# Sid-Rafilson-1617/poor-man-GPLVM

Measured on NVIDIA B200. Metric: EM time-bins x iters/s, higher is better.
Workload: dtype f32

## Files before the change

### poor_man_gplvm_b200/csrc/pmg_gemm_tc.cu

```cuda
#include "pmg_common.cuh"
#include "pmg_tc.cuh"
#include <cuda_bf16.h>

namespace pmg {

using namespace tc;

constexpr int TC_BM = 128;
constexpr int TC_BK = 64;
constexpr int TC_THREADS = 256;
constexpr int TC_A_BYTES = TC_BM * TC_BK * 2;

__global__ void counts_to_f16_kernel(int64_t T, int N, const float* __restrict__ y, int64_t ldy,
                                     __half* __restrict__ y16, int64_t ld16, int* __restrict__ inexact) {
  const int64_t total = T * ld16;
  int bad = 0;
  for (int64_t i = (int64_t)blockIdx.x * blockDim.x + threadIdx.x; i < total; i += (int64_t)gridDim.x * blockDim.x) {
    const int64_t t = i / ld16;
    const int n = (int)(i - t * ld16);
    float v = 0.f;
    if (n < N) v = y[(size_t)t * ldy + n];
    const __half h = __float2half_rn(v);
    if (__half2float(h) != v) ++bad;
    y16[i] = h;
// ... 687 lines not shown
        }
      }
    }
  } else if (warp == 1) {
    if (lane == 0) {
      int stage = 0; uint32_t phase = 0; int it = 0;
      for (int tile = blockIdx.x; tile < n_tiles; tile += gridDim.x, ++it) {
        const int buf = it & 1;
        const uint32_t acc_phase = (it >> 1) & 1;
        mbar_wait(&tempty[buf], acc_phase ^ 1);
        tc_fence_after();
        const uint32_t d_tmem = tmem_base + (uint32_t)(buf * BN);
        for (int kb = 0; kb < p.n_kblocks; ++kb) {
          mbar_wait(&full[stage], phase);
          tc_fence_after();
          const uint32_t sA = smem_u32(smem + (size_t)stage * stage_bytes);
#pragma unroll
          for (int pc = 0; pc < EM_PB; ++pc) {
            const uint32_t sB = sA + TC_A_BYTES + pc * b_bytes;
#pragma unroll
            for (int k = 0; k < TC_BK / 16; ++k) {
              const uint64_t ad = make_smem_desc(sA + k * 32, 16, 1024);
              const uint64_t bd = make_smem_desc(sB + k * 32, 16, 1024);
              mma_f16_ss(d_tmem, ad, bd, p.idesc, (kb | pc | k) != 0);
            }
          }
          mma_commit(&empty[stage]);
          if (++stage == p.stages) { stage = 0; phase ^= 1; }
        }
        mma_commit(&tfull[buf]);
      }
    }
  } else if (warp >= 4) {
    const int q = warp & 3;
    int it = 0;
    for (int tile = blockIdx.x; tile < n_tiles; tile += gridDim.x, ++it) {
      const int mt = tile / p.n_ntiles, nt = tile % p.n_ntiles;
      const int buf = it & 1;
      const uint32_t acc_phase = (it >> 1) & 1;
      mbar_wait(&tfull[buf], acc_phase);
      tc_fence_after();
      const int64_t t = (int64_t)mt * TC_BM + q * 32 + lane;
      const bool t_ok = t < p.T;
      const float lg = t_ok ? p.lgam[t] : 0.f;
      float* orow = p.ll + (size_t)(t_ok ? t : 0) * p.ldll;
      const uint32_t taddr = tmem_base + ((uint32_t)(q * 32) << 16) + (uint32_t)(buf * BN);
      const bool vec_ok = (p.ldll & 3) == 0;
      for (int c0 = 0; c0 < BN; c0 += 16) {
        uint32_t r[16];
        tmem_ld_x16(taddr + c0, r);
        tmem_ld_wait();
        const int k0 = nt * BN + c0;
        if (t_ok && k0 < p.K) {
          float v[16];
#pragma unroll
          for (int j = 0; j < 16; ++j) {
            const int k = k0 + j;
            float x = __uint_as_float(r[j]);
            if (k < p.K) {
              x = x - __ldg(p.lam_sum + k) - lg;
              if (p.ma_latent && __ldg(p.ma_latent + k) == 0.f) x = kVeryNegLL;
            }
            v[j] = x;
          }
          if (vec_ok && k0 + 16 <= p.K) {
#pragma unroll
            for (int j = 0; j < 16; j += 4)
              *reinterpret_cast<float4*>(orow + k0 + j) = make_float4(v[j], v[j + 1], v[j + 2], v[j + 3]);
          } else {
#pragma unroll
            for (int j = 0; j < 16; ++j)
              if (k0 + j < p.K) orow[k0 + j] = v[j];
          }
        }
      }
      tc_fence_before();
      mbar_arrive(&tempty[buf]);
    }
  }
  tc_fence_before();
  __syncthreads();
  if (warp == 2) { tc_fence_after(); tmem_dealloc(tmem_base, p.tmem_cols); }
}

static uint32_t pow2_cols(int c) {
  uint32_t v = 32;
  while ((int)v < c) v <<= 1;
  return v;
}

}

extern "C" int pmg_emission_tile_n(int K) {
  if (K <= 0) return 0;
  const int nt = (K + 255) / 256;
  int bn = (K + nt - 1) / nt;
  bn = (bn + 15) / 16 * 16;
  return bn;
}

extern "C" int pmg_counts_to_f16(int64_t T, int N, const float* y, int64_t ldy, void* y16, int64_t ld16,
                                 int* inexact_count, pmg_stream_t stream) {
  if (T <= 0 || N <= 0 || !y || !y16 || !inexact_count || ldy < N || ld16 < N || (ld16 & 7)) return PMG_ERR_BAD_ARG;
  cudaStream_t st = (cudaStream_t)stream;
  PMG_CUDA_CHECK(cudaMemsetAsync(inexact_count, 0, sizeof(int), st));
  pmg::counts_to_f16_kernel<<<148 * 8, 256, 0, st>>>(T, N, y, ldy, (__half*)y16, ld16, inexact_count);
  PMG_LAUNCH_CHECK();
  return PMG_OK;
}

extern "C" int pmg_counts_prepare(int64_t T, int N, const float* y, int64_t ldy, const float* ma_neuron, void* y16,
                                  int64_t ld16, int ones_col, int* inexact_count, float* lgam, float* ysum,
                                  pmg_stream_t stream) {
  if (T <= 0 || N <= 0 || !y || !y16 || !inexact_count || !lgam || ldy < N || (ld16 & 7)) return PMG_ERR_BAD_ARG;
  if (ld16 < N + (ones_col ? 1 : 0)) return PMG_ERR_BAD_ARG;
  cudaStream_t st = (cudaStream_t)stream;
  PMG_CUDA_CHECK(cudaMemsetAsync(inexact_count, 0, sizeof(int), st));
  const bool vec = (N & 3) == 0 && (ldy & 3) == 0 && ((uintptr_t)y & 15) == 0 && (!ma_neuron || ((uintptr_t)ma_neuron & 15) == 0);
  const unsigned grid = (unsigned)pmg::cdiv(T, 8);
  if (vec)
    pmg::counts_prepare_kernel<true><<<grid, 256, 0, st>>>(T, N, y, ldy, ma_neuron, (__half*)y16, ld16, ones_col,
                                                           inexact_count, lgam, ysum);
  else
    pmg::counts_prepare_kernel<false><<<grid, 256, 0, st>>>(T, N, y, ldy, ma_neuron, (__half*)y16, ld16, ones_col,
                                                            inexact_count, lgam, ysum);
  PMG_LAUNCH_CHECK();
  return PMG_OK;
}

extern "C" int pmg_counts_prepare_shifted(int64_t T, int N, int n_shift, const void* yT16, int64_t ld_src,
                                          const int* shifts, const float* ma_neuron, void* y16, int64_t ld16,
                                          float* lgam, pmg_stream_t stream) {
  if (T <= 0 || N <= 0 || n_shift <= 0 || !yT16 || !shifts || !y16 || !lgam) return PMG_ERR_BAD_ARG;
  if (ld_src < T || ld16 < N || (ld16 & 7)) return PMG_ERR_BAD_ARG;
  if ((uintptr_t)y16 & 15) return PMG_ERR_ALIGNMENT;
  const int64_t n_tiles = (T + pmg::SH_TT - 1) / pmg::SH_TT;
  if (n_tiles * n_shift > 0x7fffffffLL) return PMG_ERR_UNSUPPORTED_SHAPE;
  const bool vec = (N & 3) == 0 && (!ma_neuron || ((uintptr_t)ma_neuron & 15) == 0);
  const unsigned grid = (unsigned)(n_tiles * n_shift);
  cudaStream_t st = (cudaStream_t)stream;
  if (vec)
    pmg::counts_prepare_shifted_kernel<true><<<grid, pmg::SH_THREADS, 0, st>>>(
        T, N, n_tiles, (const __half*)yT16, ld_src, shifts, ma_neuron, (__half*)y16, ld16, lgam);
  else
    pmg::counts_prepare_shifted_kernel<false><<<grid, pmg::SH_THREADS, 0, st>>>(
        T, N, n_tiles, (const __half*)yT16, ld_src, shifts, ma_neuron, (__half*)y16, ld16, lgam);
  PMG_LAUNCH_CHECK();
  return PMG_OK;
}

extern "C" int pmg_emission_prepare_f16(int K, int N, const float* tuning, const float* ma_neuron, float dt,
                                        int Kpad, int64_t ld16, void* loglam16, float* lam_sum,
                                        pmg_stream_t stream) {
  if (K <= 0 || N <= 0 || !tuning || !loglam16 || !lam_sum || Kpad < K || ld16 < N || (ld16 & 7)) return PMG_ERR_BAD_ARG;
  pmg::emission_prepare_f16_kernel<<<Kpad, 128, 0, (cudaStream_t)stream>>>(K, N, tuning, ma_neuron, dt, Kpad, ld16,
                                                                          (__half*)loglam16, lam_sum);
  PMG_LAUNCH_CHECK();
  return PMG_OK;
}

extern "C" int pmg_emission_poisson_f16(int64_t T, int N, int K, const void* y16, int64_t ld16,
                                        const void* loglam16, int Kpad, const float* lam_sum, const float* lgam,
                                        const float* ma_latent, float* ll, int64_t ldll, pmg_stream_t stream) {
  using namespace pmg;
  if (T <= 0 || N <= 0 || K <= 0 || !y16 || !loglam16 || !lam_sum || !lgam || !ll) return PMG_ERR_BAD_ARG;
  if (ld16 < N || (ld16 & 7) || ldll < K) return PMG_ERR_BAD_ARG;
  if (((uintptr_t)y16 & 15) || ((uintptr_t)loglam16 & 15)) return PMG_ERR_ALIGNMENT;
  const int BN = pmg_emission_tile_n(K);
  const int n_ntiles = (K + BN - 1) / BN;
  if (Kpad != n_ntiles * BN) return PMG_ERR_BAD_ARG;
  if (T > ((int64_t)1 << 31) - 256) return PMG_ERR_UNSUPPORTED_SHAPE;

  CUtensorMap tmA, tmB;
  int rc = make_tmap_f16(&tmA, y16, (uint64_t)T, (uint64_t)ld16, (uint64_t)ld16, TC_BM);
  if (rc) return PMG_ERR_UNSUPPORTED_SHAPE;
  rc = make_tmap_f16(&tmB, loglam16, (uint64_t)EM_PB * Kpad, (uint64_t)ld16, (uint64_t)ld16, (uint32_t)BN);
  if (rc) return PMG_ERR_UNSUPPORTED_SHAPE;

  EmissionTcParams p;
  p.T = T; p.K = K; p.Kpad = Kpad; p.BN = BN;
  p.n_kblocks = (int)((ld16 + TC_BK - 1) / TC_BK);
  p.n_mtiles = (int)((T + TC_BM - 1) / TC_BM);
  p.n_ntiles = n_ntiles;
  p.stagger = 0;
  p.idesc = make_idesc_f16(TC_BM, BN, 0, 0, 0);
  p.tmem_cols = pow2_cols(2 * BN);
  p.lam_sum = lam_sum; p.lgam = lgam; p.ma_latent = ma_latent; p.ll = ll; p.ldll = ldll;
  p.ep_nbuf = 0;
  cudaStream_t st = (cudaStream_t)stream;
  int dev = 0, sms = 0;
  PMG_CUDA_CHECK(cudaGetDevice(&dev));
  PMG_CUDA_CHECK(cudaDeviceGetAttribute(&sms, cudaDevAttrMultiProcessorCount, dev));
  const size_t smem_max = 227 * 1024;

  bool paired = (ldll & 3) == 0 && ((uintptr_t)ll & 15) == 0;
  if (paired && (BN % 16) == 0 && T >= 4 * TC_BM) {
    const uint32_t stage_bytes = EM_MI * TC_A_BYTES + EM_PB * (BN / 2) * TC_BK * 2;
    const size_t fixed = 1024  + 256  + (size_t)((Kpad + 3) & ~3) * sizeof(float);
    int nbuf = 2, stages = 0;
    for (; nbuf >= 1; --nbuf) {
      const size_t stg_bytes = (size_t)8 * nbuf * EP_BUF_BYTES;
      stages = fixed + stg_bytes < smem_max ? (int)((smem_max - fixed - stg_bytes) / stage_bytes) : 0;
      if (stages >= 3) break;
    }
    if (nbuf < 1) { nbuf = 1; }
    if (stages >= 2) {
      if (stages > 6) stages = 6;
      EmissionTcParams p2 = p;
      p2.stages = stages;
      p2.ep_nbuf = nbuf;
      p2.idesc = make_idesc_f16(2 * TC_BM, BN, 0, 0, 0);
      CUtensorMap tmBh, tmC32, tmC16;
      rc = make_tmap_f16(&tmBh, loglam16, (uint64_t)EM_PB * Kpad, (uint64_t)ld16, (uint64_t)ld16, (uint32_t)(BN / 2));
      if (rc) return PMG_ERR_UNSUPPORTED_SHAPE;
      rc = make_tmap_f32(&tmC32, ll, (uint64_t)T, (uint64_t)K, (uint64_t)ldll, 32, 32);
      if (rc) return PMG_ERR_UNSUPPORTED_SHAPE;
      rc = make_tmap_f32(&tmC16, ll, (uint64_t)T, (uint64_t)K, (uint64_t)ldll, 32, 16);
      if (rc) return PMG_ERR_UNSUPPORTED_SHAPE;
      const size_t smem = (size_t)stages * stage_bytes + (size_t)8 * nbuf * EP_BUF_BYTES + fixed;
      PMG_CUDA_CHECK(cudaFuncSetAttribute(emission_tc2_kernel, cudaFuncAttributeMaxDynamicSharedMemorySize, (int)smem));
      PMG_CUDA_CHECK(cudaFuncSetAttribute(emission_tc2_kernel, cudaFuncAttributeNonPortableClusterSizeAllowed, 0));
      cudaLaunchConfig_t cfg = {};
      cudaLaunchAttribute attr[1];
      attr[0].id = cudaLaunchAttributeClusterDimension;
      attr[0].val.clusterDim.x = 2; attr[0].val.clusterDim.y = 1; attr[0].val.clusterDim.z = 1;
      cfg.blockDim = dim3(EM_THREADS); cfg.dynamicSmemBytes = smem; cfg.stream = st;
      cfg.attrs = attr; cfg.numAttrs = 1;
      cfg.gridDim = dim3((unsigned)(sms & ~1));
      static size_t occ_smem = 0;
      static int occ_clusters = 0, occ_dev = -1;
      static cudaError_t occ_err = cudaSuccess;
      if (occ_smem != smem || occ_dev != dev) {
        occ_dev = dev;
        occ_err = cudaOccupancyMaxActiveClusters(&occ_clusters, emission_tc2_kernel, &cfg);
        occ_smem = smem;
      }
      const int max_clusters = occ_clusters;
      const cudaError_t oe = occ_err;
      const int n_units2 = ((p.n_mtiles + 2 * EM_MI - 1) / (2 * EM_MI)) * p.n_ntiles;
      if (oe == cudaSuccess && max_clusters >= 1) {
        int n_cl = max_clusters < n_units2 ? max_clusters : n_units2;
        if (n_cl > sms / 2) n_cl = sms / 2;
        cfg.gridDim = dim3((unsigned)(2 * n_cl));
        PMG_CUDA_CHECK(cudaLaunchKernelEx(&cfg, emission_tc2_kernel, tmA, tmBh, tmC32, tmC16, p2));
        return PMG_OK;
      }
      (void)cudaGetLastError();
    }
  }
  if (paired) {
    const uint32_t stage_bytes = EM_MI * TC_A_BYTES + EM_PB * BN * TC_BK * 2;
    const size_t fixed = 1024  + 256  + (size_t)((Kpad + 3) & ~3) * sizeof(float);
    int nbuf = 2;
    int stages = 0;
    for (; nbuf >= 1; --nbuf) {
      const size_t stg_bytes = (size_t)8 * nbuf * EP_BUF_BYTES;
      stages = fixed + stg_bytes < smem_max ? (int)((smem_max - fixed - stg_bytes) / stage_bytes) : 0;
      if (stages >= 2) break;
    }
    if (stages < 2) {
      paired = false;
    } else {
      if (stages > 6) stages = 6;
      p.stages = stages;
      p.ep_nbuf = nbuf;
      CUtensorMap tmC32, tmC16;
      rc = make_tmap_f32(&tmC32, ll, (uint64_t)T, (uint64_t)K, (uint64_t)ldll, 32, 32);
      if (rc) return PMG_ERR_UNSUPPORTED_SHAPE;
      rc = make_tmap_f32(&tmC16, ll, (uint64_t)T, (uint64_t)K, (uint64_t)ldll, 32, 16);
      if (rc) return PMG_ERR_UNSUPPORTED_SHAPE;
      const size_t smem = (size_t)stages * stage_bytes + (size_t)8 * nbuf * EP_BUF_BYTES + fixed;
      PMG_CUDA_CHECK(cudaFuncSetAttribute(emission_tc_kernel, cudaFuncAttributeMaxDynamicSharedMemorySize, (int)smem));
      const int n_units = ((p.n_mtiles + EM_MI - 1) / EM_MI) * p.n_ntiles;
      emission_tc_kernel<<<n_units < sms ? n_units : sms, EM_THREADS, smem, st>>>(tmA, tmB, tmC32, tmC16, p);
      PMG_LAUNCH_CHECK();
      return PMG_OK;
    }
  }
  {
    const uint32_t stage_bytes = TC_A_BYTES + EM_PB * BN * TC_BK * 2;
    int stages = (int)((225 * 1024) / stage_bytes);
    if (stages > 2) stages = 2;
    if (stages < 2) return PMG_ERR_UNSUPPORTED_SHAPE;
    p.stages = stages;
    const size_t smem = (size_t)stages * stage_bytes + 1024  + 256 ;
    PMG_CUDA_CHECK(cudaFuncSetAttribute(emission_tc_kernel_v1, cudaFuncAttributeMaxDynamicSharedMemorySize, (int)smem));
    const int n_tiles = p.n_mtiles * p.n_ntiles;
    emission_tc_kernel_v1<<<n_tiles < sms ? n_tiles : sms, TC_THREADS, smem, st>>>(tmA, tmB, p);
    PMG_LAUNCH_CHECK();
  }
  return PMG_OK;
}

namespace pmg {

constexpr int AT_BKT = 32;
constexpr int AT_BOX_BYTES = AT_BKT * 128;
constexpr int AT_PG = 2;

struct AtbTcParams {
  int64_t T, t_per_split;
  int64_t g_lo_row;
  int K, N, BN, n_mtiles, n_ntiles, splits, stages;
  uint32_t tmem_cols;
  float* partial;
};

template <int PA, int FMT>
__global__ void __launch_bounds__(TC_THREADS, 1)
atb_tc_kernel(const __grid_constant__ CUtensorMap tmY, const __grid_constant__ CUtensorMap tmY1,
              const __grid_constant__ CUtensorMap tmG, const __grid_constant__ CUtensorMap tmG1,
              const AtbTcParams p) {
  extern __shared__ __align__(1024) uint8_t smem_raw[];
  uint8_t* smem = reinterpret_cast<uint8_t*>((reinterpret_cast<uintptr_t>(smem_raw) + 1023) & ~(uintptr_t)1023);
  const int mp = blockIdx.x, nt = blockIdx.y, sp = blockIdx.z;
  const int n_mi = (2 * mp + 1 < p.n_mtiles) ? 2 : 1;
  const int k_base = nt * p.BN;
  int bn = p.K - k_base;
  bn = (bn + 63) / 64 * 64;
  if (bn > p.BN) bn = p.BN;
  const int n_boxes_b = bn / 64;
  const uint32_t a_tile_bytes = 2 * AT_BOX_BYTES;
  const uint32_t a_bytes = 2 * PA * a_tile_bytes;
  const uint32_t b_piece_bytes = (uint32_t)(p.BN / 64) * AT_BOX_BYTES;
  const uint32_t stage_bytes = a_bytes + AT_PG * b_piece_bytes;
  uint64_t* full = reinterpret_cast<uint64_t*>(smem + (size_t)p.stages * stage_bytes);
  uint64_t* empty = full + p.stages;
  uint64_t* tfull = empty + p.stages;
  uint32_t* tmem_slot = reinterpret_cast<uint32_t*>(tfull + 1);

  const int warp = threadIdx.x >> 5, lane = threadIdx.x & 31;
  if (threadIdx.x == 0) {
    for (int s = 0; s < p.stages; ++s) { mbar_init(&full[s], 1); mbar_init(&empty[s], 1); }
    mbar_init(tfull, 1);
    fence_barrier_init();
  }
  if (warp == 0 && lane == 0) { tma_prefetch_desc(&tmY); tma_prefetch_desc(&tmG); tma_prefetch_desc(&tmG1); }
  if (warp == 2) { tmem_alloc(tmem_slot, p.tmem_cols); tmem_relinquish(); }
  tc_fence_before();
  __syncthreads();
  tc_fence_after();
  const uint32_t tmem_base = *tmem_slot;

  const int64_t t_begin = (int64_t)sp * p.t_per_split;
  int64_t t_end = t_begin + p.t_per_split;
  if (t_end > p.T) t_end = p.T;
  const int n_tb = t_end > t_begin ? (int)((t_end - t_begin + AT_BKT - 1) / AT_BKT) : 0;
  const uint32_t tx_bytes = (uint32_t)(n_mi * PA) * a_tile_bytes + AT_PG * (uint32_t)n_boxes_b * AT_BOX_BYTES;

  if (warp == 0) {
    if (lane == 0) {
      int stage = 0; uint32_t phase = 0;
      for (int tb = 0; tb < n_tb; ++tb) {
        mbar_wait(&empty[stage], phase ^ 1);
        uint8_t* sA = smem + (size_t)stage * stage_bytes;
        const int t0 = (int)(t_begin + (int64_t)tb * AT_BKT);
        mbar_arrive_expect_tx(&full[stage], tx_bytes);
        for (int mi = 0; mi < n_mi; ++mi) {
          const int m0 = (2 * mp + mi) * TC_BM;
#pragma unroll
          for (int pa = 0; pa < PA; ++pa) {
            const CUtensorMap* tm = pa == 0 ? &tmY : &tmY1;
            uint8_t* dst = sA + (mi * PA + pa) * a_tile_bytes;
            tma_load_2d(dst, tm, &full[stage], m0, t0);
            tma_load_2d(dst + AT_BOX_BYTES, tm, &full[stage], m0 + 64, t0);
          }
        }
        for (int pc = 0; pc < AT_PG; ++pc)
          for (int b = 0; b < n_boxes_b; ++b)
            tma_load_2d(sA + a_bytes + pc * b_piece_bytes + b * AT_BOX_BYTES, pc == 0 ? &tmG : &tmG1, &full[stage],
                        k_base + b * 64, (int)(pc * p.g_lo_row) + t0);
        if (++stage == p.stages) { stage = 0; phase ^= 1; }
      }
    }
  } else if (warp == 1) {
    if (lane == 0) {
      const uint32_t idesc = make_idesc_f16(TC_BM, bn, 1, 1, FMT);
      int stage = 0; uint32_t phase = 0;
      for (int tb = 0; tb < n_tb; ++tb) {
        mbar_wait(&full[stage], phase);
        tc_fence_after();
        const uint32_t sA = smem_u32(smem + (size_t)stage * stage_bytes);
        for (int mi = 0; mi < n_mi; ++mi) {
#pragma unroll
          for (int pa = 0; pa < PA; ++pa) {
#pragma unroll
            for (int pc = 0; pc < AT_PG; ++pc) {
              if (pa + pc > 1) continue;
              const uint32_t sB = sA + a_bytes + pc * b_piece_bytes;
#pragma unroll
              for (int k = 0; k < AT_BKT / 16; ++k) {
                const uint64_t ad = make_smem_desc(sA + (mi * PA + pa) * a_tile_bytes + k * 2048, AT_BOX_BYTES, 1024);
                const uint64_t bd = make_smem_desc(sB + k * 2048, AT_BOX_BYTES, 1024);
                mma_f16_ss(tmem_base + (uint32_t)(mi * p.BN), ad, bd, idesc, (tb | pa | pc | k) != 0);
              }
            }
          }
        }
        mma_commit(&empty[stage]);
        if (++stage == p.stages) { stage = 0; phase ^= 1; }
      }
      mma_commit(tfull);
    }
  } else if (warp >= 4) {
    const int q = warp & 3;
    float* out = p.partial + (size_t)sp * p.K * p.N;
    if (n_tb > 0) {
      mbar_wait(tfull, 0);
      tc_fence_after();
    }
    for (int mi = 0; mi < n_mi; ++mi) {
      const int n = (2 * mp + mi) * TC_BM + q * 32 + lane;
      const uint32_t taddr = tmem_base + ((uint32_t)(q * 32) << 16) + (uint32_t)(mi * p.BN);
      for (int c0 = 0; c0 < bn; c0 += 16) {
        uint32_t r[16];
        if (n_tb > 0) {
          tmem_ld_x16(taddr + c0, r);
          tmem_ld_wait();
        } else {
#pragma unroll
          for (int j = 0; j < 16; ++j) r[j] = 0u;
        }
        if (n < p.N) {
#pragma unroll
          for (int j = 0; j < 16; ++j) {
            const int k = k_base + c0 + j;
            if (k < p.K) out[(size_t)k * p.N + n] = __uint_as_float(r[j]);
          }
        }
      }
    }
  }
  tc_fence_before();
  __syncthreads();
  if (warp == 2) { tc_fence_after(); tmem_dealloc(tmem_base, p.tmem_cols); }
}

__global__ void split_bf16_kernel(int64_t T, int K, const float* __restrict__ src, int64_t lds,
                                  __nv_bfloat16* __restrict__ dst, int64_t ld16) {
  const int64_t total = T * ld16;
  for (int64_t i = (int64_t)blockIdx.x * blockDim.x + threadIdx.x; i < total; i += (int64_t)gridDim.x * blockDim.x) {
    const int64_t t = i / ld16;
    const int k = (int)(i - t * ld16);
    const float v = k < K ? src[(size_t)t * lds + k] : 0.f;
    const __nv_bfloat16 h = __float2bfloat16_rn(v);
    dst[i] = h;
    dst[total + i] = __float2bfloat16_rn(v - __bfloat162float(h));
  }
}

template <int HALF>
__global__ void __launch_bounds__(256) split_pieces_vec_kernel(int64_t T, int K8, const float* __restrict__ src,
                                                               int64_t lds, uint16_t* __restrict__ dst, int64_t ld16) {
  const int64_t total = T * (int64_t)K8;
  const size_t piece = (size_t)T * ld16;
  for (int64_t g = (int64_t)blockIdx.x * blockDim.x + threadIdx.x; g < total; g += (int64_t)gridDim.x * blockDim.x) {
    const int64_t t = g / K8;
    const int k = (int)(g - t * K8) * 8;
    const float4* sp = reinterpret_cast<const float4*>(src + (size_t)t * lds + k);
    const float4 a = __ldcs(sp), b = __ldcs(sp + 1);
    const float v[8] = {a.x, a.y, a.z, a.w, b.x, b.y, b.z, b.w};
    uint16_t hi[8], lo[8];
#pragma unroll
    for (int e = 0; e < 8; ++e) {
      if (HALF) {
        const __half h = __float2half_rn(v[e]);
        hi[e] = __half_as_ushort(h);
        lo[e] = __half_as_ushort(__float2half_rn(v[e] - __half2float(h)));
      } else {
        const __nv_bfloat16 h = __float2bfloat16_rn(v[e]);
        hi[e] = __bfloat16_as_ushort(h);
        lo[e] = __bfloat16_as_ushort(__float2bfloat16_rn(v[e] - __bfloat162float(h)));
      }
    }
    uint4 H, L;
    H.x = hi[0] | ((uint32_t)hi[1] << 16); H.y = hi[2] | ((uint32_t)hi[3] << 16);
    H.z = hi[4] | ((uint32_t)hi[5] << 16); H.w = hi[6] | ((uint32_t)hi[7] << 16);
    L.x = lo[0] | ((uint32_t)lo[1] << 16); L.y = lo[2] | ((uint32_t)lo[3] << 16);
    L.z = lo[4] | ((uint32_t)lo[5] << 16); L.w = lo[6] | ((uint32_t)lo[7] << 16);
    uint16_t* o = dst + (size_t)t * ld16 + k;
    *reinterpret_cast<uint4*>(o) = H;
    *reinterpret_cast<uint4*>(o + piece) = L;
  }
}

static bool split_vec_ok(int K, const void* src, int64_t lds, const void* dst, int64_t ld16) {
  return (K % 8) == 0 && K == ld16 && (lds % 4) == 0 && (((uintptr_t)src | (uintptr_t)dst) & 15) == 0;
}

__global__ void split_f16_kernel(int64_t T, int K, const float* __restrict__ src, int64_t lds,
                                 __half* __restrict__ dst, int64_t ld16) {
  const int64_t total = T * ld16;
  for (int64_t i = (int64_t)blockIdx.x * blockDim.x + threadIdx.x; i < total; i += (int64_t)gridDim.x * blockDim.x) {
    const int64_t t = i / ld16;
    const int k = (int)(i - t * ld16);
    const float v = k < K ? src[(size_t)t * lds + k] : 0.f;
    const __half h = __float2half_rn(v);
    dst[i] = h;
    dst[total + i] = __float2half_rn(v - __half2float(h));
  }
}

__global__ void split_reduce_kernel_tc(int splits, int64_t MN, const float* __restrict__ partial,
                                       float* __restrict__ C) {
  const int64_t i = (int64_t)blockIdx.x * blockDim.x + threadIdx.x;
  if (i >= MN) return;
  double s = 0.0;
  for (int z = 0; z < splits; ++z) s += (double)partial[(size_t)z * MN + i];
  C[i] = (float)s;
}

static void atb_tc_plan(int64_t T, int K, int N, int& BN, int& n_mtiles, int& n_ntiles, int& splits,
                        int64_t& t_per_split) {
  BN = K >= 256 ? 256 : (K + 63) / 64 * 64;
  n_ntiles = (K + BN - 1) / BN;
  n_mtiles = (N + TC_BM - 1) / TC_BM;
  const int tiles = ((n_mtiles + 1) / 2) * n_ntiles;
  splits = 148 / tiles;
  if (splits < 1) splits = 1;
  const int64_t max_splits = (T + 4 * AT_BKT - 1) / (4 * AT_BKT);
  if (splits > max_splits) splits = (int)max_splits;
  if (splits < 1) splits = 1;
  t_per_split = ((T + splits - 1) / splits + AT_BKT - 1) / AT_BKT * AT_BKT;
  splits = (int)((T + t_per_split - 1) / t_per_split);
}

}

extern "C" int pmg_split_f16(int64_t T, int K, const float* src, int64_t lds, void* dst16, int64_t ld16,
                             pmg_stream_t stream) {
  if (T <= 0 || K <= 0 || !src || !dst16 || lds < K || ld16 < K || (ld16 & 7)) return PMG_ERR_BAD_ARG;
  if (pmg::split_vec_ok(K, src, lds, dst16, ld16))
    pmg::split_pieces_vec_kernel<1><<<148 * 16, 256, 0, (cudaStream_t)stream>>>(T, K / 8, src, lds, (uint16_t*)dst16, ld16);
  else
    pmg::split_f16_kernel<<<148 * 8, 256, 0, (cudaStream_t)stream>>>(T, K, src, lds, (__half*)dst16, ld16);
  PMG_LAUNCH_CHECK();
  return PMG_OK;
}

extern "C" int64_t pmg_atb_f16_workspace_bytes(int64_t T, int K, int N) {
  if (T <= 0 || K <= 0 || N <= 0) return 0;
  int BN, nm, nn, splits; int64_t tps;
  pmg::atb_tc_plan(T, K, N, BN, nm, nn, splits, tps);
  return (int64_t)splits * K * N * (int64_t)sizeof(float);
}

extern "C" int pmg_split_bf16(int64_t T, int K, const float* src, int64_t lds, void* dst16, int64_t ld16,
                              pmg_stream_t stream) {
  if (T <= 0 || K <= 0 || !src || !dst16 || lds < K || ld16 < K || (ld16 & 7)) return PMG_ERR_BAD_ARG;
  if (pmg::split_vec_ok(K, src, lds, dst16, ld16))
    pmg::split_pieces_vec_kernel<0><<<148 * 16, 256, 0, (cudaStream_t)stream>>>(T, K / 8, src, lds, (uint16_t*)dst16, ld16);
  else
    pmg::split_bf16_kernel<<<148 * 8, 256, 0, (cudaStream_t)stream>>>(T, K, src, lds, (__nv_bfloat16*)dst16, ld16);
  PMG_LAUNCH_CHECK();
  return PMG_OK;
}

static int atb_pieces_launch(int64_t T, int K, int N, const void* g16, const void* g16_lo, int64_t ldg,
                             const void* y16, const void* y16_lo, int64_t ldy16, int fmt, float* yw, void* workspace,
                             int64_t workspace_bytes, pmg_stream_t stream);

extern "C" int pmg_atb_f16(int64_t T, int K, int N, const void* g16, int64_t ldg, const void* y16, int64_t ldy16,
                           float* yw, void* workspace, int64_t workspace_bytes, pmg_stream_t stream) {
  return atb_pieces_launch(T, K, N, g16, nullptr, ldg, y16, nullptr, ldy16, 0, yw, workspace, workspace_bytes, stream);
}

extern "C" int pmg_atb_bf16x2(int64_t T, int K, int N, const void* g16, int64_t ldg, const void* y16, int64_t ldy16,
                              float* out, void* workspace, int64_t workspace_bytes, pmg_stream_t stream) {
  if (!y16 || T <= 0) return PMG_ERR_BAD_ARG;
  const char* lo = (const char*)y16 + (size_t)T * (size_t)ldy16 * 2;
  return atb_pieces_launch(T, K, N, g16, nullptr, ldg, y16, lo, ldy16, 1, out, workspace, workspace_bytes, stream);
}

extern "C" int pmg_atb_bf16x2_pieces(int64_t T, int K, int N, const void* g_hi, const void* g_lo, int64_t ldg,
                                     const void* y_hi, const void* y_lo, int64_t ldy16, float* out, void* workspace,
                                     int64_t workspace_bytes, pmg_stream_t stream) {
  if (!g_hi || !g_lo || !y_hi || !y_lo || T <= 0) return PMG_ERR_BAD_ARG;
  return atb_pieces_launch(T, K, N, g_hi, g_lo, ldg, y_hi, y_lo, ldy16, 1, out, workspace, workspace_bytes, stream);
}

static int atb_pieces_launch(int64_t T, int K, int N, const void* g16, const void* g16_lo, int64_t ldg,
                             const void* y16, const void* y16_lo, int64_t ldy16, int fmt, float* yw, void* workspace,
                             int64_t workspace_bytes, pmg_stream_t stream) {
  using namespace pmg;
  if (T <= 0 || K <= 0 || N <= 0 || !g16 || !y16 || !yw) return PMG_ERR_BAD_ARG;
  if (ldg < K || (ldg & 7) || ldy16 < N || (ldy16 & 7)) return PMG_ERR_BAD_ARG;
  if (((uintptr_t)g16 & 15) || ((uintptr_t)y16 & 15) || ((uintptr_t)g16_lo & 15)) return PMG_ERR_ALIGNMENT;
  if ((int64_t)AT_PG * T > ((int64_t)1 << 31) - 256) return PMG_ERR_UNSUPPORTED_SHAPE;
  AtbTcParams p;
  atb_tc_plan(T, K, N, p.BN, p.n_mtiles, p.n_ntiles, p.splits, p.t_per_split);
  if (!workspace || workspace_bytes < (int64_t)p.splits * K * N * (int64_t)sizeof(float)) return PMG_ERR_WORKSPACE;
  p.T = T; p.K = K; p.N = N; p.partial = (float*)workspace;
  const int PA = y16_lo ? 2 : 1;
  if (y16_lo && ((uintptr_t)y16_lo & 15)) return PMG_ERR_ALIGNMENT;
  const uint32_t stage_bytes = 4 * PA * AT_BOX_BYTES + AT_PG * (p.BN / 64) * AT_BOX_BYTES;
  int stages = (int)((200 * 1024) / stage_bytes);
  if (stages > 8) stages = 8;
  if (stages < 2) return PMG_ERR_UNSUPPORTED_SHAPE;
  p.stages = stages;
  p.tmem_cols = pow2_cols(2 * p.BN);

  CUtensorMap tmY, tmY1, tmG, tmG1;
  int rc = make_tmap_f16(&tmY, y16, (uint64_t)T, (uint64_t)ldy16, (uint64_t)ldy16, AT_BKT);
  if (rc) return PMG_ERR_UNSUPPORTED_SHAPE;
  rc = make_tmap_f16(&tmY1, y16_lo ? y16_lo : y16, (uint64_t)T, (uint64_t)ldy16, (uint64_t)ldy16, AT_BKT);
  if (rc) return PMG_ERR_UNSUPPORTED_SHAPE;
  rc = make_tmap_f16(&tmG, g16, (uint64_t)(g16_lo ? 1 : AT_PG) * T, (uint64_t)ldg, (uint64_t)ldg, AT_BKT);
  if (rc) return PMG_ERR_UNSUPPORTED_SHAPE;
  tmG1 = tmG;
  p.g_lo_row = T;
  if (g16_lo) {
    rc = make_tmap_f16(&tmG1, g16_lo, (uint64_t)T, (uint64_t)ldg, (uint64_t)ldg, AT_BKT);
    if (rc) return PMG_ERR_UNSUPPORTED_SHAPE;
    p.g_lo_row = 0;
  }
  const size_t smem = (size_t)stages * stage_bytes + 1024 + 256;
  cudaStream_t st = (cudaStream_t)stream;
  dim3 grid((p.n_mtiles + 1) / 2, p.n_ntiles, p.splits);
  if (PA == 1 && fmt == 0) {
    PMG_CUDA_CHECK(cudaFuncSetAttribute(atb_tc_kernel<1, 0>, cudaFuncAttributeMaxDynamicSharedMemorySize, (int)smem));
    atb_tc_kernel<1, 0><<<grid, TC_THREADS, smem, st>>>(tmY, tmY1, tmG, tmG1, p);
  } else if (PA == 2 && fmt == 1) {
    PMG_CUDA_CHECK(cudaFuncSetAttribute(atb_tc_kernel<2, 1>, cudaFuncAttributeMaxDynamicSharedMemorySize, (int)smem));
    atb_tc_kernel<2, 1><<<grid, TC_THREADS, smem, st>>>(tmY, tmY1, tmG, tmG1, p);
  } else {
    return PMG_ERR_BAD_ARG;
  }
  PMG_LAUNCH_CHECK();
  const int64_t MN = (int64_t)K * N;
  split_reduce_kernel_tc<<<cdiv(MN, 256), 256, 0, st>>>(p.splits, MN, p.partial, yw);
  PMG_LAUNCH_CHECK();
  return PMG_OK;
}

int64_t pmg_atb_tc_workspace_bytes(int64_t, int, int) { return 0; }
int pmg_atb_tc_launch(int64_t, int, int, const float*, int64_t, const float*, int64_t, float*, int64_t, void*,
                      int64_t, cudaStream_t) {
  return PMG_ERR_UNSUPPORTED_SHAPE;
}
```

### poor_man_gplvm_b200/csrc/pmg_tc.cuh

```cuda
#pragma once
#include <cuda.h>
#include <cuda_fp16.h>
#include <cuda_runtime.h>
#include <stdint.h>

namespace pmg {
namespace tc {

__device__ __forceinline__ uint32_t smem_u32(const void* p) {
  return static_cast<uint32_t>(__cvta_generic_to_shared(p));
}

__device__ __forceinline__ void mbar_init(uint64_t* bar, uint32_t count) {
  asm volatile("mbarrier.init.shared::cta.b64 [%0], %1;" ::"r"(smem_u32(bar)), "r"(count) : "memory");
}
__device__ __forceinline__ void fence_barrier_init() {
  asm volatile("fence.mbarrier_init.release.cluster;" ::: "memory");
}
__device__ __forceinline__ void mbar_arrive_expect_tx(uint64_t* bar, uint32_t bytes) {
  asm volatile("mbarrier.arrive.expect_tx.shared::cta.b64 _, [%0], %1;" ::"r"(smem_u32(bar)), "r"(bytes)
               : "memory");
}
__device__ __forceinline__ void mbar_arrive(uint64_t* bar) {
  asm volatile("mbarrier.arrive.shared::cta.b64 _, [%0];" ::"r"(smem_u32(bar)) : "memory");
}
__device__ __forceinline__ bool mbar_try_wait(uint64_t* bar, uint32_t parity) {
  uint32_t ok;
  asm volatile(
      "{\n\t.reg .pred p;\n\t"
      "mbarrier.try_wait.parity.shared::cta.b64 p, [%1], %2;\n\t"
      "selp.u32 %0, 1, 0, p;\n\t}"
      : "=r"(ok)
      : "r"(smem_u32(bar)), "r"(parity)
      : "memory");
  return ok != 0;
}
__device__ __forceinline__ void mbar_wait(uint64_t* bar, uint32_t parity) {
  while (!mbar_try_wait(bar, parity)) { }
}

__device__ __forceinline__ void tma_prefetch_desc(const CUtensorMap* m) {
  asm volatile("prefetch.tensormap [%0];" ::"l"(reinterpret_cast<uint64_t>(m)) : "memory");
}
__device__ __forceinline__ void tma_load_2d(void* smem_dst, const CUtensorMap* m, uint64_t* bar, int c_inner,
                                            int c_outer) {
  asm volatile(
      "cp.async.bulk.tensor.2d.shared::cluster.global.mbarrier::complete_tx::bytes [%0], [%1, {%3, %4}], [%2];"
      ::"r"(smem_u32(smem_dst)), "l"(reinterpret_cast<uint64_t>(m)), "r"(smem_u32(bar)), "r"(c_inner), "r"(c_outer)
      : "memory");
}

__device__ __forceinline__ void tma_store_2d(const CUtensorMap* m, const void* smem_src, int c_inner, int c_outer) {
  asm volatile("cp.async.bulk.tensor.2d.global.shared::cta.bulk_group [%0, {%2, %3}], [%1];"
               ::"l"(reinterpret_cast<uint64_t>(m)), "r"(smem_u32(smem_src)), "r"(c_inner), "r"(c_outer)
               : "memory");
}
__device__ __forceinline__ void bulk_commit() { asm volatile("cp.async.bulk.commit_group;" ::: "memory"); }
template <int N>
__device__ __forceinline__ void bulk_wait_read() {
  asm volatile("cp.async.bulk.wait_group.read %0;" ::"n"(N) : "memory");
}
__device__ __forceinline__ void fence_proxy_async_smem() { asm volatile("fence.proxy.async.shared::cta;" ::: "memory"); }

__device__ __forceinline__ void tmem_alloc(uint32_t* smem_dst, uint32_t ncols) {
  asm volatile("tcgen05.alloc.cta_group::1.sync.aligned.shared::cta.b32 [%0], %1;" ::"r"(smem_u32(smem_dst)),
               "r"(ncols)
               : "memory");
}
__device__ __forceinline__ void tmem_relinquish() {
  asm volatile("tcgen05.relinquish_alloc_permit.cta_group::1.sync.aligned;" ::: "memory");
}
__device__ __forceinline__ void tmem_dealloc(uint32_t taddr, uint32_t ncols) {
  asm volatile("tcgen05.dealloc.cta_group::1.sync.aligned.b32 %0, %1;" ::"r"(taddr), "r"(ncols) : "memory");
}
__device__ __forceinline__ void tc_fence_before() { asm volatile("tcgen05.fence::before_thread_sync;" ::: "memory"); }
__device__ __forceinline__ void tc_fence_after() { asm volatile("tcgen05.fence::after_thread_sync;" ::: "memory"); }

__device__ __forceinline__ void mma_f16_ss(uint32_t d_tmem, uint64_t adesc, uint64_t bdesc, uint32_t idesc,
                                           uint32_t accumulate) {
  asm volatile(
      "{\n\t.reg .pred p;\n\t"
      "setp.ne.b32 p, %4, 0;\n\t"
      "tcgen05.mma.cta_group::1.kind::f16 [%0], %1, %2, %3, p;\n\t}"
      ::"r"(d_tmem), "l"(adesc), "l"(bdesc), "r"(idesc), "r"(accumulate)
      : "memory");
}
__device__ __forceinline__ void mma_commit(uint64_t* bar) {
  asm volatile("tcgen05.commit.cta_group::1.mbarrier::arrive::one.shared::cluster.b64 [%0];" ::"r"(smem_u32(bar))
               : "memory");
}
__device__ __forceinline__ void tmem_ld_x16(uint32_t taddr, uint32_t (&r)[16]) {
  asm volatile(
      "tcgen05.ld.sync.aligned.32x32b.x16.b32 {%0, %1, %2, %3, %4, %5, %6, %7, %8, %9, %10, %11, %12, %13, %14, %15}, "
      "[%16];"
      : "=r"(r[0]), "=r"(r[1]), "=r"(r[2]), "=r"(r[3]), "=r"(r[4]), "=r"(r[5]), "=r"(r[6]), "=r"(r[7]), "=r"(r[8]),
        "=r"(r[9]), "=r"(r[10]), "=r"(r[11]), "=r"(r[12]), "=r"(r[13]), "=r"(r[14]), "=r"(r[15])
      : "r"(taddr)
      : "memory");
}
__device__ __forceinline__ void tmem_ld_x16_of32(uint32_t taddr, uint32_t (&r)[32]) {
  asm volatile(
      "tcgen05.ld.sync.aligned.32x32b.x16.b32 {%0, %1, %2, %3, %4, %5, %6, %7, %8, %9, %10, %11, %12, %13, %14, %15}, "
      "[%16];"
      : "=r"(r[0]), "=r"(r[1]), "=r"(r[2]), "=r"(r[3]), "=r"(r[4]), "=r"(r[5]), "=r"(r[6]), "=r"(r[7]), "=r"(r[8]),
        "=r"(r[9]), "=r"(r[10]), "=r"(r[11]), "=r"(r[12]), "=r"(r[13]), "=r"(r[14]), "=r"(r[15])
      : "r"(taddr)
      : "memory");
}
__device__ __forceinline__ void tmem_ld_x32(uint32_t taddr, uint32_t (&r)[32]) {
  asm volatile(
      "tcgen05.ld.sync.aligned.32x32b.x32.b32 {%0, %1, %2, %3, %4, %5, %6, %7, %8, %9, %10, %11, %12, %13, %14, %15, "
      "%16, %17, %18, %19, %20, %21, %22, %23, %24, %25, %26, %27, %28, %29, %30, %31}, [%32];"
      : "=r"(r[0]), "=r"(r[1]), "=r"(r[2]), "=r"(r[3]), "=r"(r[4]), "=r"(r[5]), "=r"(r[6]), "=r"(r[7]), "=r"(r[8]),
        "=r"(r[9]), "=r"(r[10]), "=r"(r[11]), "=r"(r[12]), "=r"(r[13]), "=r"(r[14]), "=r"(r[15]), "=r"(r[16]),
        "=r"(r[17]), "=r"(r[18]), "=r"(r[19]), "=r"(r[20]), "=r"(r[21]), "=r"(r[22]), "=r"(r[23]), "=r"(r[24]),
        "=r"(r[25]), "=r"(r[26]), "=r"(r[27]), "=r"(r[28]), "=r"(r[29]), "=r"(r[30]), "=r"(r[31])
      : "r"(taddr)
      : "memory");
}
__device__ __forceinline__ void tmem_ld_wait() { asm volatile("tcgen05.wait::ld.sync.aligned;" ::: "memory"); }

__device__ __forceinline__ uint32_t cluster_ctarank() {
  uint32_t r;
  asm volatile("mov.u32 %0, %%cluster_ctarank;" : "=r"(r));
  return r;
}
__device__ __forceinline__ void cluster_sync_all() {
  asm volatile("barrier.cluster.arrive.release.aligned;\n\tbarrier.cluster.wait.acquire.aligned;" ::: "memory");
}
__device__ __forceinline__ void tmem_alloc2(uint32_t* smem_dst, uint32_t ncols) {
  asm volatile("tcgen05.alloc.cta_group::2.sync.aligned.shared::cta.b32 [%0], %1;" ::"r"(smem_u32(smem_dst)),
               "r"(ncols)
               : "memory");
}
__device__ __forceinline__ void tmem_relinquish2() {
  asm volatile("tcgen05.relinquish_alloc_permit.cta_group::2.sync.aligned;" ::: "memory");
}
__device__ __forceinline__ void tmem_dealloc2(uint32_t taddr, uint32_t ncols) {
  asm volatile("tcgen05.dealloc.cta_group::2.sync.aligned.b32 %0, %1;" ::"r"(taddr), "r"(ncols) : "memory");
}
__device__ __forceinline__ void mma_f16_ss2(uint32_t d_tmem, uint64_t adesc, uint64_t bdesc, uint32_t idesc,
                                            uint32_t accumulate) {
  const uint32_t z = 0;
  asm volatile(
      "{\n\t.reg .pred p;\n\t"
      "setp.ne.b32 p, %4, 0;\n\t"
      "tcgen05.mma.cta_group::2.kind::f16 [%0], %1, %2, %3, {%5, %5, %5, %5, %5, %5, %5, %5}, p;\n\t}"
      ::"r"(d_tmem), "l"(adesc), "l"(bdesc), "r"(idesc), "r"(accumulate), "r"(z)
      : "memory");
}
__device__ __forceinline__ void mma_commit2(uint64_t* bar, uint16_t cta_mask) {
  asm volatile("tcgen05.commit.cta_group::2.mbarrier::arrive::one.shared::cluster.multicast::cluster.b64 [%0], %1;"
               ::"r"(smem_u32(bar)), "h"(cta_mask)
               : "memory");
}
__device__ __forceinline__ void tma_load_2d_pair(void* smem_dst, const CUtensorMap* m, uint64_t* bar, int c_inner,
                                                 int c_outer) {
  asm volatile(
      "cp.async.bulk.tensor.2d.cta_group::2.shared::cluster.global.mbarrier::complete_tx::bytes [%0], [%1, {%3, %4}], [%2];"
      ::"r"(smem_u32(smem_dst)), "l"(reinterpret_cast<uint64_t>(m)), "r"(smem_u32(bar) & 0xFEFFFFFFu), "r"(c_inner),
        "r"(c_outer)
      : "memory");
}
__device__ __forceinline__ void mbar_arrive_cluster(uint64_t* bar, uint32_t cta) {
  asm volatile(
      "{\n\t.reg .b32 ra;\n\t"
      "mapa.shared::cluster.u32 ra, %0, %1;\n\t"
      "mbarrier.arrive.release.cluster.shared::cluster.b64 _, [ra];\n\t}"
      ::"r"(smem_u32(bar)), "r"(cta)
      : "memory");
}

__device__ __forceinline__ uint64_t make_smem_desc(uint32_t saddr, uint32_t lbo_bytes, uint32_t sbo_bytes) {
  uint64_t d = 0;
  d |= (uint64_t)((saddr >> 4) & 0x3FFF);
  d |= (uint64_t)((lbo_bytes >> 4) & 0x3FFF) << 16;
  d |= (uint64_t)((sbo_bytes >> 4) & 0x3FFF) << 32;
  d |= (uint64_t)1 << 46;
  d |= (uint64_t)2 << 61;
  return d;
}
__host__ __device__ constexpr uint32_t make_idesc_f16(int M, int N, int a_mn_major, int b_mn_major, int fmt) {
  return (1u << 4) | ((uint32_t)fmt << 7) | ((uint32_t)fmt << 10) | ((uint32_t)a_mn_major << 15) |
         ((uint32_t)b_mn_major << 16) | ((uint32_t)(N >> 3) << 17) | ((uint32_t)(M >> 4) << 24);
}

}

typedef CUresult (*PFN_encodeTiled)(CUtensorMap*, CUtensorMapDataType, cuuint32_t, void*, const cuuint64_t*,
                                    const cuuint64_t*, const cuuint32_t*, const cuuint32_t*, CUtensorMapInterleave,
                                    CUtensorMapSwizzle, CUtensorMapL2promotion, CUtensorMapFloatOOBfill);

inline PFN_encodeTiled get_encode_tiled() {
  static PFN_encodeTiled fn = nullptr;
  if (!fn) {
    void* p = nullptr;
    cudaDriverEntryPointQueryResult q;
    if (cudaGetDriverEntryPoint("cuTensorMapEncodeTiled", &p, cudaEnableDefault, &q) == cudaSuccess &&
        q == cudaDriverEntryPointSuccess)
      fn = reinterpret_cast<PFN_encodeTiled>(p);
  }
  return fn;
}

inline int make_tmap_f16(CUtensorMap* map, const void* base, uint64_t rows, uint64_t cols, uint64_t ld,
                         uint32_t box_rows) {
  PFN_encodeTiled enc = get_encode_tiled();
  if (!enc) return -100;
  cuuint64_t gdim[2] = {cols, rows};
  cuuint64_t gstr[1] = {ld * 2};
  cuuint32_t box[2] = {64, box_rows};
  cuuint32_t estr[2] = {1, 1};
  CUresult r = enc(map, CU_TENSOR_MAP_DATA_TYPE_FLOAT16, 2, const_cast<void*>(base), gdim, gstr, box, estr,
                   CU_TENSOR_MAP_INTERLEAVE_NONE, CU_TENSOR_MAP_SWIZZLE_128B, CU_TENSOR_MAP_L2_PROMOTION_L2_256B,
                   CU_TENSOR_MAP_FLOAT_OOB_FILL_NONE);
  return r == CUDA_SUCCESS ? 0 : -101;
}

inline int make_tmap_f32(CUtensorMap* map, const void* base, uint64_t rows, uint64_t cols, uint64_t ld,
                         uint32_t box_rows, uint32_t box_cols) {
  PFN_encodeTiled enc = get_encode_tiled();
  if (!enc) return -100;
  cuuint64_t gdim[2] = {cols, rows};
  cuuint64_t gstr[1] = {ld * 4};
  cuuint32_t box[2] = {box_cols, box_rows};
  cuuint32_t estr[2] = {1, 1};
  const CUtensorMapSwizzle sw = box_cols * 4 == 128 ? CU_TENSOR_MAP_SWIZZLE_128B
                              : box_cols * 4 == 64 ? CU_TENSOR_MAP_SWIZZLE_64B : CU_TENSOR_MAP_SWIZZLE_NONE;
  CUresult r = enc(map, CU_TENSOR_MAP_DATA_TYPE_FLOAT32, 2, const_cast<void*>(base), gdim, gstr, box, estr,
                   CU_TENSOR_MAP_INTERLEAVE_NONE, sw, CU_TENSOR_MAP_L2_PROMOTION_NONE,
                   CU_TENSOR_MAP_FLOAT_OOB_FILL_NONE);
  return r == CUDA_SUCCESS ? 0 : -101;
}

}
```

Baseline: 283.2 million.

## Multicast G tiles across 2-CTA clusters in atb kernel and balance BN tiling

Launches the A^T·B tensor-core kernel as 2-CTA clusters when they fit. Each CTA loads half of the shared G pieces via TMA multicast to both CTAs, and the empty barriers now wait on commits from both CTAs' MMAs, which cuts duplicate global/L2 traffic for the B operand. The plan also picks BN as an even split of K rounded to 16 instead of fixed 256/64 granularity, reducing padded MMA columns. This adds cluster synchronisation and cross-CTA coupling, plus an occupancy query cached in host statics.

```diff
diff --git a/poor_man_gplvm_b200/csrc/pmg_gemm_tc.cu b/poor_man_gplvm_b200/csrc/pmg_gemm_tc.cu
--- a/poor_man_gplvm_b200/csrc/pmg_gemm_tc.cu
+++ b/poor_man_gplvm_b200/csrc/pmg_gemm_tc.cu
@@ -1013,6 +1013,7 @@
   int64_t T, t_per_split;
   int64_t g_lo_row;
   int K, N, BN, n_mtiles, n_ntiles, splits, stages;
+  int pair;
   uint32_t tmem_cols;
   float* partial;
 };
@@ -1028,12 +1029,12 @@
   const int n_mi = (2 * mp + 1 < p.n_mtiles) ? 2 : 1;
   const int k_base = nt * p.BN;
   int bn = p.K - k_base;
-  bn = (bn + 63) / 64 * 64;
+  bn = (bn + 15) / 16 * 16;
   if (bn > p.BN) bn = p.BN;
-  const int n_boxes_b = bn / 64;
+  const int n_boxes_b = (bn + 63) / 64;
   const uint32_t a_tile_bytes = 2 * AT_BOX_BYTES;
   const uint32_t a_bytes = 2 * PA * a_tile_bytes;
-  const uint32_t b_piece_bytes = (uint32_t)(p.BN / 64) * AT_BOX_BYTES;
+  const uint32_t b_piece_bytes = (uint32_t)((p.BN + 63) / 64) * AT_BOX_BYTES;
   const uint32_t stage_bytes = a_bytes + AT_PG * b_piece_bytes;
   uint64_t* full = reinterpret_cast<uint64_t*>(smem + (size_t)p.stages * stage_bytes);
   uint64_t* empty = full + p.stages;
@@ -1042,15 +1043,16 @@
 
   const int warp = threadIdx.x >> 5, lane = threadIdx.x & 31;
   if (threadIdx.x == 0) {
-    for (int s = 0; s < p.stages; ++s) { mbar_init(&full[s], 1); mbar_init(&empty[s], 1); }
+    for (int s = 0; s < p.stages; ++s) { mbar_init(&full[s], 1); mbar_init(&empty[s], p.pair ? 2 : 1); }
     mbar_init(tfull, 1);
     fence_barrier_init();
   }
   if (warp == 0 && lane == 0) { tma_prefetch_desc(&tmY); tma_prefetch_desc(&tmG); tma_prefetch_desc(&tmG1); }
   if (warp == 2) { tmem_alloc(tmem_slot, p.tmem_cols); tmem_relinquish(); }
   tc_fence_before();
-  __syncthreads();
+  cluster_sync_all();
   tc_fence_after();
+  const int rank = p.pair ? (int)cluster_ctarank() : 0;
   const uint32_t tmem_base = *tmem_slot;
 
   const int64_t t_begin = (int64_t)sp * p.t_per_split;
@@ -1077,10 +1079,16 @@
             tma_load_2d(dst + AT_BOX_BYTES, tm, &full[stage], m0 + 64, t0);
           }
         }
-        for (int pc = 0; pc < AT_PG; ++pc)
-          for (int b = 0; b < n_boxes_b; ++b)
-            tma_load_2d(sA + a_bytes + pc * b_piece_bytes + b * AT_BOX_BYTES, pc == 0 ? &tmG : &tmG1, &full[stage],
-                        k_base + b * 64, (int)(pc * p.g_lo_row) + t0);
+        for (int pc = 0; pc < AT_PG; ++pc) {
+          if (p.pair && pc != rank) continue;
+          for (int b = 0; b < n_boxes_b; ++b) {
+            uint8_t* dst = sA + a_bytes + pc * b_piece_bytes + b * AT_BOX_BYTES;
+            const CUtensorMap* tm = pc == 0 ? &tmG : &tmG1;
+            const int row = (int)(pc * p.g_lo_row) + t0;
+            if (p.pair) tma_load_2d_mc(dst, tm, &full[stage], k_base + b * 64, row, 3);
+            else tma_load_2d(dst, tm, &full[stage], k_base + b * 64, row);
+          }
+        }
         if (++stage == p.stages) { stage = 0; phase ^= 1; }
       }
     }
@@ -1108,7 +1116,7 @@
             }
           }
         }
-        mma_commit(&empty[stage]);
+        if (p.pair) mma_commit_mc(&empty[stage], 3); else mma_commit(&empty[stage]);
         if (++stage == p.stages) { stage = 0; phase ^= 1; }
       }
       mma_commit(tfull);
@@ -1143,7 +1151,7 @@
     }
   }
   tc_fence_before();
-  __syncthreads();
+  cluster_sync_all();
   if (warp == 2) { tc_fence_after(); tmem_dealloc(tmem_base, p.tmem_cols); }
 }
 
@@ -1223,7 +1231,8 @@
 
 static void atb_tc_plan(int64_t T, int K, int N, int& BN, int& n_mtiles, int& n_ntiles, int& splits,
                         int64_t& t_per_split) {
-  BN = K >= 256 ? 256 : (K + 63) / 64 * 64;
+  n_ntiles = (K + 255) / 256;
+  BN = ((K + n_ntiles - 1) / n_ntiles + 15) / 16 * 16;
   n_ntiles = (K + BN - 1) / BN;
   n_mtiles = (N + TC_BM - 1) / TC_BM;
   const int tiles = ((n_mtiles + 1) / 2) * n_ntiles;
@@ -1304,7 +1313,7 @@
   p.T = T; p.K = K; p.N = N; p.partial = (float*)workspace;
   const int PA = y16_lo ? 2 : 1;
   if (y16_lo && ((uintptr_t)y16_lo & 15)) return PMG_ERR_ALIGNMENT;
-  const uint32_t stage_bytes = 4 * PA * AT_BOX_BYTES + AT_PG * (p.BN / 64) * AT_BOX_BYTES;
+  const uint32_t stage_bytes = 4 * PA * AT_BOX_BYTES + AT_PG * ((p.BN + 63) / 64) * AT_BOX_BYTES;
   int stages = (int)((200 * 1024) / stage_bytes);
   if (stages > 8) stages = 8;
   if (stages < 2) return PMG_ERR_UNSUPPORTED_SHAPE;
@@ -1328,15 +1337,40 @@
   const size_t smem = (size_t)stages * stage_bytes + 1024 + 256;
   cudaStream_t st = (cudaStream_t)stream;
   dim3 grid((p.n_mtiles + 1) / 2, p.n_ntiles, p.splits);
-  if (PA == 1 && fmt == 0) {
-    PMG_CUDA_CHECK(cudaFuncSetAttribute(atb_tc_kernel<1, 0>, cudaFuncAttributeMaxDynamicSharedMemorySize, (int)smem));
-    atb_tc_kernel<1, 0><<<grid, TC_THREADS, smem, st>>>(tmY, tmY1, tmG, tmG1, p);
-  } else if (PA == 2 && fmt == 1) {
-    PMG_CUDA_CHECK(cudaFuncSetAttribute(atb_tc_kernel<2, 1>, cudaFuncAttributeMaxDynamicSharedMemorySize, (int)smem));
-    atb_tc_kernel<2, 1><<<grid, TC_THREADS, smem, st>>>(tmY, tmY1, tmG, tmG1, p);
-  } else {
-    return PMG_ERR_BAD_ARG;
-  }
+  void (*kern)(const CUtensorMap, const CUtensorMap, const CUtensorMap, const CUtensorMap, const AtbTcParams);
+  if (PA == 1 && fmt == 0) kern = atb_tc_kernel<1, 0>;
+  else if (PA == 2 && fmt == 1) kern = atb_tc_kernel<2, 1>;
+  else return PMG_ERR_BAD_ARG;
+  PMG_CUDA_CHECK(cudaFuncSetAttribute(kern, cudaFuncAttributeMaxDynamicSharedMemorySize, (int)smem));
+  cudaLaunchConfig_t cfg = {};
+  cudaLaunchAttribute attr[1];
+  attr[0].id = cudaLaunchAttributeClusterDimension;
+  attr[0].val.clusterDim.x = 2; attr[0].val.clusterDim.y = 1; attr[0].val.clusterDim.z = 1;
+  cfg.gridDim = grid; cfg.blockDim = dim3(TC_THREADS); cfg.dynamicSmemBytes = smem; cfg.stream = st;
+  cfg.attrs = attr; cfg.numAttrs = 1;
+  p.pair = 0;
+  if (grid.x % 2 == 0) {
+    int dev = 0, sms = 0;
+    PMG_CUDA_CHECK(cudaGetDevice(&dev));
+    PMG_CUDA_CHECK(cudaDeviceGetAttribute(&sms, cudaDevAttrMultiProcessorCount, dev));
+    const int n_ctas = (int)(grid.x * grid.y * grid.z);
+    if (n_ctas <= sms) {
+      static size_t occ_smem[2] = {0, 0};
+      static int occ_clusters[2] = {0, 0}, occ_dev[2] = {-1, -1};
+      const int ki = PA == 1 ? 0 : 1;
+      if (occ_smem[ki] != smem || occ_dev[ki] != dev) {
+        occ_dev[ki] = dev;
+        occ_smem[ki] = smem;
+        if (cudaOccupancyMaxActiveClusters(&occ_clusters[ki], kern, &cfg) != cudaSuccess) {
+          occ_clusters[ki] = 0;
+          (void)cudaGetLastError();
+        }
+      }
+      p.pair = occ_clusters[ki] >= n_ctas / 2;
+    }
+  }
+  if (!p.pair) cfg.numAttrs = 0;
+  PMG_CUDA_CHECK(cudaLaunchKernelEx(&cfg, kern, tmY, tmY1, tmG, tmG1, p));
   PMG_LAUNCH_CHECK();
   const int64_t MN = (int64_t)K * N;
   split_reduce_kernel_tc<<<cdiv(MN, 256), 256, 0, st>>>(p.splits, MN, p.partial, yw);
diff --git a/poor_man_gplvm_b200/csrc/pmg_tc.cuh b/poor_man_gplvm_b200/csrc/pmg_tc.cuh
--- a/poor_man_gplvm_b200/csrc/pmg_tc.cuh
+++ b/poor_man_gplvm_b200/csrc/pmg_tc.cuh
@@ -161,6 +161,20 @@
       ::"r"(smem_u32(smem_dst)), "l"(reinterpret_cast<uint64_t>(m)), "r"(smem_u32(bar) & 0xFEFFFFFFu), "r"(c_inner),
         "r"(c_outer)
       : "memory");
+}
+__device__ __forceinline__ void tma_load_2d_mc(void* smem_dst, const CUtensorMap* m, uint64_t* bar, int c_inner,
+                                               int c_outer, uint16_t cta_mask) {
+  asm volatile(
+      "cp.async.bulk.tensor.2d.shared::cluster.global.mbarrier::complete_tx::bytes.multicast::cluster"
+      " [%0], [%1, {%3, %4}], [%2], %5;"
+      ::"r"(smem_u32(smem_dst)), "l"(reinterpret_cast<uint64_t>(m)), "r"(smem_u32(bar)), "r"(c_inner), "r"(c_outer),
+        "h"(cta_mask)
+      : "memory");
+}
+__device__ __forceinline__ void mma_commit_mc(uint64_t* bar, uint16_t cta_mask) {
+  asm volatile("tcgen05.commit.cta_group::1.mbarrier::arrive::one.shared::cluster.multicast::cluster.b64 [%0], %1;"
+               ::"r"(smem_u32(bar)), "h"(cta_mask)
+               : "memory");
 }
 __device__ __forceinline__ void mbar_arrive_cluster(uint64_t* bar, uint32_t cta) {
   asm volatile(
```

Result: faster. 291.8 million (median of 6 runs) (+3.1%).
